# timmeinhardt/trackformer

Measured on AMD Instinct MI355X. Metric: frames/sec, TrackFormer-Deformable inference (ResNet-50, 1333x800, 300 object + 100 track queries, bs 1 per GPU); roofline = ms_deform_attn HBM GB/s, higher is better.
Workload: dtype f32 (dense layers as the fp16 split product on MFMA: two fp16 pieces per activation, three per weight scaled per output channel -- 22 + 1 significand bits per operand, the one dropped product < 2^-22 --, three terms, f32 accumulate)

## Files before the change

include/tf_fused.h:

```cpp
#ifndef TF_FUSED_H_
#define TF_FUSED_H_

#include <stdint.h>

#ifdef __cplusplus
extern "C" {
#endif

int tf_bias_act_f32(float *x, const float *bias, const float *residual, int64_t n, int C, int relu,
                    void *stream);

int tf_add_layernorm_f32(const float *x, const float *res, const float *gamma, const float *beta,
                         float *out, int64_t rows, int C, float eps, void *stream);

int tf_box_refine_f32(const float *delta, const float *ref, float *out, int64_t rows, int ref_dim, float eps, void *stream);

int tf_postprocess_pack_f32(const float *logits, const float *boxes, float *out, int64_t Q, int C, float img_h, float img_w,
                            int clip, void *stream);

int tf_groupnorm_nhwc_f32(const float *x, const float *gamma, const float *beta, float *out, double *workspace, int N,
                          int HW, int C, int G, float eps, int64_t x_image_stride, int64_t out_image_stride, void *stream);
int tf_groupnorm_stats_nhwc_f32(const float *x, double *workspace, int N, int HW, int C, int G, int64_t x_image_stride, void *stream);
int tf_groupnorm_relu_nhwc_f32(const float *x, const float *gamma, const float *beta, float *out, double *workspace, int N,
                               int HW, int C, int G, float eps, int64_t x_image_stride, int64_t out_image_stride, void *stream);
// ... 108 lines not shown
int tf_conv_packed_f32(const float *x, const void *w_packed, const float *bias, const float *residual, float *y, float *workspace,
                       int ksplit, int nimg, int hin, int win, int cin, int cout, int ks, int stride, int relu, int terms,
                       void *stream);
int tf_conv_packed_partials_f32(const float *x, const void *w_packed, const float *bias, float *workspace, int ksplit, int nimg, int hin,
                                int win, int cin, int cout, int ks, int stride, int terms, int *pieces, void *stream);

int tf_linear_res_ln_f32(const float *x, const void *w_packed, const float *bias, const float *residual, const float *ln_weight,
                         const float *ln_bias, float ln_eps, float *y, int64_t M, int K, int N, int terms, void *stream);

int tf_ffn_fused_f32(const float *x, const void *w1_packed, const float *b1, const void *w2_packed, const float *b2,
                     const float *residual, const float *ln_weight, const float *ln_bias, float ln_eps, float *y, int64_t M,
                     int d_model, int d_ffn, int terms, void *stream);

typedef struct tf_proj_group {
    const void *w_packed;
    const float *bias;
    float *y;
    int N;
    int add_x2;
} tf_proj_group;
int tf_linear_groups_f32(const float *x, const float *x2, const tf_proj_group *groups, int ngroups, int64_t M, int K, int terms,
                         void *stream);

int tf_mha_core_f32(const float *q, const float *k, const float *v, float *out, const unsigned char *key_mask,
                    int N, int Lq, int Lk, int H, int D, int ldq, int ldk, int ldv, int ldo, float scale,
                    void *stream);

int tf_mha_core_train_f32(const float *q, const float *k, const float *v, float *out, const unsigned char *key_mask, float *stats,
                          const int64_t *rng, float p, int N, int Lq, int Lk, int H, int D, int ldq, int ldk, int ldv, int ldo,
                          float scale, void *stream);
int tf_mha_core_bwd_f32(const float *dout, const float *q, const float *k, const float *v, const float *out, const float *stats,
                        const unsigned char *key_mask, const int64_t *rng, float p, float *dq, float *dk, float *dv, int N, int Lq,
                        int Lk, int H, int D, int lddo, int ldq, int ldk, int ldv, int ldo, int lddq, int lddk, int lddv, float scale,
                        void *stream);

int tf_nms_host_f32(const float *boxes, const float *scores, int n, float iou_threshold, int64_t *keep, int *n_keep);

#ifdef __cplusplus
}
#endif
#endif
```

include/tf_msda.h:

```cpp
#ifndef TF_MSDA_H_
#define TF_MSDA_H_

#include <stdint.h>

#ifdef __cplusplus
extern "C" {
#endif

#define TF_MSDA_ABI_VERSION 12
#define TF_MSDA_MAX_LEVELS 16

typedef enum tf_msda_status {
    TF_MSDA_OK = 0,
    TF_MSDA_ERR_NULL_POINTER = -1,
    TF_MSDA_ERR_BAD_DIMS = -2,
    TF_MSDA_ERR_SHAPE_SUM = -3,
    TF_MSDA_ERR_LAUNCH = -4,
    TF_MSDA_ERR_NO_DEVICE = -5,
    TF_MSDA_ERR_WORKSPACE = -6
} tf_msda_status;

int tf_msda_abi_version(void);

const char *tf_msda_strerror(int status);

int tf_msda_last_hip_error(void);

const char *tf_msda_last_kernel(void);

int tf_msda_set_tiled(int mode);

int tf_msda_set_option(const char *name, int value);
// ... 79 lines not shown
```

trackformer_amd/build.py:

```python
import hashlib
import os
import shutil
import subprocess
import sys
from concurrent.futures import ThreadPoolExecutor

PKG_DIR = os.path.dirname(os.path.abspath(__file__))
REPO_DIR = os.path.dirname(PKG_DIR)
CSRC = os.path.join(PKG_DIR, "csrc")
LIB_DIR = os.path.join(PKG_DIR, "lib")
INCLUDE = os.path.join(REPO_DIR, "include")
GFX_ARCH = "gfx950"

_TARGETS = [
    ("libtf_msda.so", ["msda_hip.hip", "msda_pquad.hip", "fused_ops.hip", "linear_split.hip", "linear_stream.hip", "mha_core.hip", "ffn_fused.hip", "stem_conv.hip", "msda_host.cpp"], []),
]


def _hipcc():
    exe = shutil.which("hipcc") or "/opt/rocm/bin/hipcc"
    if not os.path.exists(exe):
        raise RuntimeError("hipcc not found (expected on PATH or at /opt/rocm/bin/hipcc)")
    return exe

# ... 37 lines not shown
        src_paths = [os.path.join(CSRC, s) for s in srcs]
        flags = ["--offload-arch=" + GFX_ARCH, "-O3", "-std=c++17", "-fPIC", "-I" + INCLUDE,
                 "-Wno-pass-failed"] + extra
        key = _key(src_paths + headers, flags)
        if not force and not _stale(out, key):
            continue
        obj_dir = os.path.join(LIB_DIR, "obj")
        os.makedirs(obj_dir, exist_ok=True)
        objs = [os.path.join(obj_dir, os.path.splitext(s)[0] + ".o") for s in srcs]
        with ThreadPoolExecutor(max_workers=len(srcs)) as pool:
            list(pool.map(lambda so: _run([_hipcc()] + flags + ["-c", so[0], "-o", so[1]], verbose),
                          zip(src_paths, objs)))
        _run([_hipcc(), "--offload-arch=" + GFX_ARCH, "-shared", "-fPIC", "-pthread"] + objs + ["-o", out], verbose)
        _stamp(out, key)
        built.append(out)
    built += _build_tools(force, verbose)
    return built


def _build_tools(force, verbose):
    out_dir = os.path.join(REPO_DIR, "tools", "bin")
    lib = os.path.join(LIB_DIR, "libtf_msda.so")
    built = []
    for name in ("msda_bench", "linear_bench", "ffn_bench", "proj_groups_bench", "gn_levels_bench"):
        src = os.path.join(REPO_DIR, "tools", name + ".cpp")
        if not os.path.exists(src):
            continue
        os.makedirs(out_dir, exist_ok=True)
        out = os.path.join(out_dir, name)
        flags = ["--offload-arch=" + GFX_ARCH, "-O2", "-std=c++17", "-I" + INCLUDE]
        headers = [os.path.join(INCLUDE, f) for f in os.listdir(INCLUDE) if f.endswith(".h")]
        key = _key([src] + headers, flags)
        if not force and not _stale(out, key) and os.path.getmtime(out) >= os.path.getmtime(lib):
            continue
        _run([_hipcc()] + flags + [src, "-L" + LIB_DIR, "-ltf_msda",
                                   "-Wl,-rpath,$ORIGIN/../../trackformer_amd/lib", "-o", out], verbose)
        _stamp(out, key)
        built.append(out)
    return built


if __name__ == "__main__":
    res = build_all(force="--force" in sys.argv, verbose=True)
    print("built:" if res else "up to date", *res)
```

trackformer_amd/csrc/ffn_fused.hip:

```cpp
#include <hip/hip_runtime.h>

#include <stdint.h>
#include <stdlib.h>

#include <type_traits>

#include "host_dispatch.h"
#include "launch_status.h"
#include "msda_common.h"
#include "split_product.h"
#include "tf_fused.h"
#include "tf_msda.h"

namespace {

template <int D>
struct Geo {
    static_assert(D == 256 || D == 288, "hidden sizes of the reference's configurations");
    static constexpr int NW = D == 256 ? 4 : 3;
    static constexpr int NT = NW * 64;
    static constexpr int TJ = D / 32 / NW;
    static constexpr int XS = D + 8;
    static constexpr int CH = NW * 32;
    static constexpr int HS = CH + 8;
// ... 654 lines not shown
        }
#pragma unroll 1
        for (int k = 0; k < pg.nchunk[ph][1]; ++k, ++ci) {
            const ChunkW nxt = chunk_of(pg.chunk[min(ci + 1, total - 1)]);
            run_chunk(std::true_type{}, cur, nxt, pg.chunk[ci]);
            cur = nxt;
        }
    }
}

template <int SP, int TI>
int launch_groups(const float *x, const float *x2, int M, const ProjGroups &pg, hipStream_t s)
{
    constexpr size_t tile = linln_lds_bytes<256>(TI, Split<SP>::NA), lds_max = tile + 2 * 4 * kMaxProjCols;
    static_assert(lds_max <= 160 * 1024, "the activation tile and the tables do not fit the LDS of a CU");
    const size_t lds = tile + 2 * 4 * (size_t)pg.ncols;
    const void *fn = (const void *)&linear_groups_kernel<SP, TI>;
    if (lds_max > 64 * 1024 && !tfm::raise_dynamic_lds_limit(fn)) return tfm::record_hip(hipErrorInvalidValue);
    const int blocks = (M + 32 * TI - 1) / (32 * TI);
    void *argv[] = {(void *)&x, (void *)&x2, (void *)&M, (void *)&pg};
    return tfm::record_hip(hipLaunchKernel(fn, dim3((unsigned)blocks), dim3(256), argv, lds, s));
}

}

extern "C" int tf_linear_groups_f32(const float *x, const float *x2, const tf_proj_group *groups, int ngroups, int64_t M, int K, int terms,
                                    void *stream)
{
    if (!x || !groups) return TF_MSDA_ERR_NULL_POINTER;
    if (ngroups < 1 || ngroups > kMaxProjGroups) return TF_MSDA_ERR_BAD_DIMS;
    for (int i = 0; i < ngroups; ++i)
        if (!groups[i].w_packed || !groups[i].y || (groups[i].add_x2 && !x2)) return TF_MSDA_ERR_NULL_POINTER;
    const int sp = split_scheme(terms);
    if (M <= 0 || K != 256 || sp == 0 || (M + 128) * (int64_t)K * 4 > 0xFFFFFFFFLL) return TF_MSDA_ERR_BAD_DIMS;
    uintptr_t al = reinterpret_cast<uintptr_t>(x) | reinterpret_cast<uintptr_t>(x2);
    ProjGroups pg{};
    for (int pass = 0; pass < 2; ++pass)
        for (int i = 0; i < ngroups; ++i) {
            const tf_proj_group &g = groups[i];
            if ((g.add_x2 != 0) != (pass == 1)) continue;
            if (g.N <= 0 || (g.N % 32) != 0 || (M + 128) * (int64_t)g.N * 4 > 0xFFFFFFFFLL) return TF_MSDA_ERR_BAD_DIMS;
            al |= reinterpret_cast<uintptr_t>(g.w_packed) | reinterpret_cast<uintptr_t>(g.bias) | reinterpret_cast<uintptr_t>(g.y);
            pg.g[pg.ng++] = ProjGroup{static_cast<const u32x4 *>(g.w_packed), g.bias, g.y, g.N, pg.ncols};
            pg.ncols += (g.N + 255) / 256 * 256;
            if (pass == 0) pg.nplain = pg.ng;
        }
    if ((al & 15) || pg.ncols > kMaxProjCols) return TF_MSDA_ERR_BAD_DIMS;
    int nc = 0;
    for (int ph = 0; ph < 2; ++ph)
        for (int half = 0; half < 2; ++half)
            for (int gi = ph ? pg.nplain : 0; gi < (ph ? pg.ng : pg.nplain); ++gi) {
                const int N = pg.g[gi].N, full_end = N / 256 * 256;
                for (int col0 = half ? full_end : 0; col0 < (half ? N : full_end); col0 += half ? 128 : 256) {
                    pg.chunk[nc++] = gi << 16 | half << 15 | col0 / 128;
                    ++pg.nchunk[ph][half];
                }
            }
    hipStream_t s = static_cast<hipStream_t>(stream);
    if (sp == 3) return launch_groups<3, 1>(x, x2, (int)M, pg, s);
    const int forced = tfm::dense_knob(tfm::kKnobGroupsTi);
    switch (forced ? forced : (M < 4096 ? 1 : 3)) {
    case 1: return launch_groups<16, 1>(x, x2, (int)M, pg, s);
    case 2: return launch_groups<16, 2>(x, x2, (int)M, pg, s);
    default: return launch_groups<16, 3>(x, x2, (int)M, pg, s);
    }
}

extern "C" int tf_linear_res_ln_f32(const float *x, const void *w_packed, const float *bias, const float *residual,
                                    const float *ln_weight, const float *ln_bias, float ln_eps, float *y, int64_t M, int K, int N,
                                    int terms, void *stream)
{
    if (!x || !w_packed || !y) return TF_MSDA_ERR_NULL_POINTER;
    if ((ln_weight == nullptr) != (ln_bias == nullptr)) return TF_MSDA_ERR_NULL_POINTER;
    const int sp = split_scheme(terms);
    if (M <= 0 || K != N || (K != 256 && K != 288) || (M + 128) * (int64_t)K * 4 > 0xFFFFFFFFLL || sp == 0) return TF_MSDA_ERR_BAD_DIMS;
    uintptr_t al = reinterpret_cast<uintptr_t>(x) | reinterpret_cast<uintptr_t>(w_packed) | reinterpret_cast<uintptr_t>(y) |
                   reinterpret_cast<uintptr_t>(bias) | reinterpret_cast<uintptr_t>(residual) | reinterpret_cast<uintptr_t>(ln_weight) |
                   reinterpret_cast<uintptr_t>(ln_bias);
    if (al & 15) return TF_MSDA_ERR_BAD_DIMS;
    const u32x4 *w = static_cast<const u32x4 *>(w_packed);
// ... 1 lines not shown
    return K == 256 ? dispatch_linln_scheme<256>(sp, x, w, bias, residual, ln_weight, ln_bias, ln_eps, y, (int)M, s)
                    : dispatch_linln_scheme<288>(sp, x, w, bias, residual, ln_weight, ln_bias, ln_eps, y, (int)M, s);
}

extern "C" int tf_ffn_fused_f32(const float *x, const void *w1_packed, const float *b1, const void *w2_packed, const float *b2,
                                const float *residual, const float *ln_weight, const float *ln_bias, float ln_eps, float *y,
                                int64_t M, int d_model, int d_ffn, int terms, void *stream)
{
    if (!x || !w1_packed || !w2_packed || !y) return TF_MSDA_ERR_NULL_POINTER;
    if ((ln_weight == nullptr) != (ln_bias == nullptr)) return TF_MSDA_ERR_NULL_POINTER;
    const int sp = split_scheme(terms);
    if (M <= 0 || (d_model != 256 && d_model != 288) || d_ffn <= 0 || sp == 0 ||
        (M + 128) * (int64_t)d_model * 4 > 0xFFFFFFFFLL)
        return TF_MSDA_ERR_BAD_DIMS;
    uintptr_t al = reinterpret_cast<uintptr_t>(x) | reinterpret_cast<uintptr_t>(w1_packed) | reinterpret_cast<uintptr_t>(w2_packed) |
                   reinterpret_cast<uintptr_t>(y) | reinterpret_cast<uintptr_t>(b1) | reinterpret_cast<uintptr_t>(b2) |
                   reinterpret_cast<uintptr_t>(residual) | reinterpret_cast<uintptr_t>(ln_weight) | reinterpret_cast<uintptr_t>(ln_bias);
    if (al & 15) return TF_MSDA_ERR_BAD_DIMS;
    const u32x4 *w1 = static_cast<const u32x4 *>(w1_packed), *w2 = static_cast<const u32x4 *>(w2_packed);
    hipStream_t s = static_cast<hipStream_t>(stream);
    return d_model == 256 ? dispatch_ffn_scheme<256>(sp, x, w1, b1, w2, b2, residual, ln_weight, ln_bias, ln_eps, y, (int)M, d_ffn, s)
                          : dispatch_ffn_scheme<288>(sp, x, w1, b1, w2, b2, residual, ln_weight, ln_bias, ln_eps, y, (int)M, d_ffn, s);
}
```

trackformer_amd/deformable_transformer.py:

```python
import copy
import math

import torch
import torch.nn.functional as F
from torch import nn
from torch.nn.init import constant_, normal_, xavier_uniform_

from . import fused
from .msda import MSDeformAttn, attach_host_shapes
from .nested import inverse_sigmoid, is_all_valid


def _inference(module) -> bool:
    return (not module.training) and (not torch.is_grad_enabled())


def _ffn_hidden(linear, activation, x, inference):
    if inference and activation is F.relu and x.is_cuda and x.dtype == torch.float32:
        if fused.split_linear_enabled():
            y = fused.linear(x, linear.weight, linear.bias, relu=True)
            if y is not None:
                return y
        x2 = x.reshape(-1, x.shape[-1])
        y = torch._addmm_activation(linear.bias, x2, linear.weight.t(), use_gelu=False)
# ... 308 lines not shown
            return (hs, memory, init_reference_out, inter_references, enc_outputs_class,
                    enc_outputs_coord_unact)
        return hs, memory, init_reference_out, inter_references, None, None


class DeformableTransformerEncoderLayer(nn.Module):
    def __init__(self, d_model=256, d_ffn=1024, dropout=0.1, activation="relu", n_levels=4,
                 n_heads=8, n_points=4):
        super().__init__()
        self.self_attn = MSDeformAttn(d_model, n_levels, n_heads, n_points)
        self.dropout1 = nn.Dropout(dropout)
        self.norm1 = nn.LayerNorm(d_model)
        self.linear1 = nn.Linear(d_model, d_ffn)
        self.activation = _get_activation_fn(activation)
        self.dropout2 = nn.Dropout(dropout)
        self.linear2 = nn.Linear(d_ffn, d_model)
        self.dropout3 = nn.Dropout(dropout)
        self.norm2 = nn.LayerNorm(d_model)

    @staticmethod
    def with_pos_embed(tensor, pos):
        return tensor if pos is None else tensor + pos

    def forward_ffn(self, src):
        inf = _inference(self)
        if inf and fused.ffn_fused_enabled() and self.activation is F.relu:
            out = fused.ffn(src, self.linear1, self.linear2, self.norm2, residual=src)
            if out is not None:
                return out
        src2 = fused.module_linear(self.linear2, _ffn_hidden_dropped(self.linear1, self.activation, src, inf, self.dropout2), inf)
        return fused.residual_norm(src, src2, self.norm2, inf, dropout=self.dropout3)

    def forward(self, src, pos, reference_points, spatial_shapes, padding_mask=None):
        inf = _inference(self)
        q, q_pos = (src, pos) if (inf and pos is not None and fused.pos_add_fused_enabled()) else (self.with_pos_embed(src, pos), None)
        if inf and fused.linear_ln_fused_enabled():
            src = self.self_attn(q, reference_points, src, spatial_shapes, padding_mask,
                                 residual_norm=(src, self.norm1), query_pos=q_pos)
            return self.forward_ffn(src)
        src2 = self.self_attn(q, reference_points, src, spatial_shapes, padding_mask, query_pos=q_pos)
        src = fused.residual_norm(src, src2, self.norm1, _inference(self), dropout=self.dropout1)
        return self.forward_ffn(src)


class DeformableTransformerEncoder(nn.Module):
    def __init__(self, encoder_layer, num_layers):
        super().__init__()
        self.layers = _get_clones(encoder_layer, num_layers)
        self.num_layers = num_layers

    @staticmethod
    def get_reference_points(spatial_shapes, valid_ratios, device):
        if torch.is_tensor(spatial_shapes):
            spatial_shapes = _host_shapes(spatial_shapes)
        per_level = []
        for lvl, (h, w) in enumerate(spatial_shapes):
            ys = torch.linspace(0.5, h - 0.5, h, dtype=torch.float32, device=device)
            xs = torch.linspace(0.5, w - 0.5, w, dtype=torch.float32, device=device)
            ref_y, ref_x = torch.meshgrid(ys, xs, indexing="ij")
            ref_y = ref_y.reshape(-1)[None] / (valid_ratios[:, None, lvl, 1] * h)
            ref_x = ref_x.reshape(-1)[None] / (valid_ratios[:, None, lvl, 0] * w)
            per_level.append(torch.stack((ref_x, ref_y), -1))
        reference_points = torch.cat(per_level, 1)
        return reference_points[:, :, None] * valid_ratios[:, None]

    def forward(self, src, spatial_shapes, valid_ratios, pos=None, padding_mask=None,
                unit_ratios=False):
        reference_points = _GEOMETRY.encoder_reference_points(
            _host_shapes(spatial_shapes), valid_ratios, unit_ratios)
        output = src
        for layer in self.layers:
            output = layer(output, pos, reference_points, spatial_shapes, padding_mask)
        return output


class DeformableTransformerDecoderLayer(nn.Module):
    def __init__(self, d_model=256, d_ffn=1024, dropout=0.1, activation="relu", n_levels=4,
                 n_heads=8, n_points=4):
        super().__init__()
        self.cross_attn = MSDeformAttn(d_model, n_levels, n_heads, n_points)
        self.dropout1 = nn.Dropout(dropout)
        self.norm1 = nn.LayerNorm(d_model)
        self.self_attn = nn.MultiheadAttention(d_model, n_heads, dropout=dropout)
        self.dropout2 = nn.Dropout(dropout)
        self.norm2 = nn.LayerNorm(d_model)
        self.linear1 = nn.Linear(d_model, d_ffn)
        self.activation = _get_activation_fn(activation)
        self.dropout3 = nn.Dropout(dropout)
        self.linear2 = nn.Linear(d_ffn, d_model)
        self.dropout4 = nn.Dropout(dropout)
        self.norm3 = nn.LayerNorm(d_model)

    @staticmethod
    def with_pos_embed(tensor, pos):
        return tensor if pos is None else tensor + pos
# ... 173 lines not shown
```

trackformer_amd/fused.py:

```python
import ctypes
import os
import threading

import torch
import torch.nn.functional as F

from . import _cabi


def _stream(device):
    return torch.cuda.current_stream(device).cuda_stream


def _param_ok(t, x):
    return (t.device == x.device and t.dtype == torch.float32 and t.is_contiguous()
            and t.data_ptr() % 16 == 0)


_weight_epoch = 0
_route_epoch = 0


def weight_epoch():
    return _weight_epoch
# ... 610 lines not shown
    if (a.data_ptr() | _ptr(b)) & 15:
        return None
    cols = 0
    for w, bias, _add in groups:
        if not (w.dtype == torch.float32 and w.dim() == 2 and w.is_contiguous() and w.device == x.device and w.shape[1] == K
                and w.shape[0] % 32 == 0 and (M + 128) * w.shape[0] * 4 <= 0xFFFFFFFF):
            return None
        if bias is not None and not (_param_ok(bias, x) and bias.numel() == w.shape[0]):
            return None
        cols += (w.shape[0] + 255) // 256 * 256
    if cols > 4096:
        return None
    packed = [_packed_weight(w, None) for w, _b, _add in groups]
    if any(p is None for p in packed):
        return None
    descs = (_cabi.ProjGroup * len(groups))()
    with torch.cuda.device(x.device):
        ys = [torch.empty((M, w.shape[0]), dtype=torch.float32, device=x.device) for w, _b, _add in groups]
        for d, (w, bias, add), p, y in zip(descs, groups, packed, ys):
            d.w_packed, d.bias, d.y, d.N, d.add_x2 = p.data_ptr(), (bias.data_ptr() if bias is not None else None), y.data_ptr(), w.shape[0], int(bool(add))
        rc = _cabi.lib().tf_linear_groups_f32(a.data_ptr(), _ptr(b) or None, descs, len(groups), M, K, _terms(), _stream(x.device))
    _cabi.check(rc, "tf_linear_groups_f32")
    return [y.view(*x.shape[:-1], y.shape[1]) for y in ys]


def conv3x3(x, w_taps, bias, relu, stride):
    if not (_split_linear and x.is_cuda and x.dtype == torch.float32 and x.dim() == 4
            and x.is_contiguous(memory_format=torch.channels_last) and w_taps.dtype == torch.float32
            and w_taps.dim() == 2 and w_taps.is_contiguous() and w_taps.device == x.device):
        return None
    n, cin, h, w = x.shape
    cout = w_taps.shape[0]
    ks = 3 if w_taps.shape[1] == 9 * cin else 1
    if w_taps.shape[1] != ks * ks * cin or cin % 32 or stride not in (1, 2) or x.numel() == 0:
        return None
    if bias is not None and not (bias.dtype == torch.float32 and bias.is_contiguous() and bias.numel() == cout
                                 and bias.device == x.device):
        return None
    pad = 1 if ks == 3 else 0
    ho, wo = (h + 2 * pad - ks) // stride + 1, (w + 2 * pad - ks) // stride + 1
    cin_ok = cin % 64 == 0 or (ks == 3 and stride == 1 and _conv_halo and cin % 32 == 0)
    stream_route = (_conv_stream and _conv_stream_wins(n * ho * wo, cout) and cin_ok and not (x.data_ptr() & 15)
                    and n * h * w * cin * 4 < 0xC0000000 and (n * ho * wo + 256) * cout * 4 < 0xC0000000)
    halo = ks == 3 and stride == 1 and _conv_halo and stream_route
    ksplit = _conv_ksplit(n * ho * wo, ks * ks * cin, cout, _HALO_KSPLIT_POLICY if halo else None)
    if ks == 1 and (ksplit < _CONV1X1_MIN_PIECES or not _conv1x1_splitk):
# ... 1317 lines not shown
```

trackformer_amd/msda.py:

```python
import ctypes
import math

import torch
import torch.nn.functional as F
from torch import nn
from torch.autograd import Function
from torch.autograd.function import once_differentiable
from torch.nn.init import constant_, xavier_uniform_

from . import _cabi, fused

import os as _os

FUSED_INFERENCE = _os.environ.get("TF_MSDA_FUSED", "1") != "0"

_HOST_SHAPE_ATTR = "_tf_msda_host_shapes"
_shape_array_cache = {}


def attach_host_shapes(spatial_shapes, host_shapes):
    setattr(spatial_shapes, _HOST_SHAPE_ATTR, tuple((int(h), int(w)) for h, w in host_shapes))
    return spatial_shapes


# ... 356 lines not shown
        self.output_proj = nn.Linear(d_model, d_model)
        self._cat_proj = _CatProjection()
        self._reset_parameters()

    def _reset_parameters(self):
        with torch.no_grad():
            constant_(self.sampling_offsets.weight, 0.)
        dirs = [(a, b) for a in (-1, 0, 1) for b in (-1, 0, 1) if (a, b) != (0, 0)]
        if self.n_heads != len(dirs):
            raise ValueError("MSDeformAttn bias initialisation requires n_heads == 8")
        grid = torch.tensor(dirs, dtype=torch.float32).view(self.n_heads, 1, 1, 2)
        grid = grid.repeat(1, self.n_levels, self.n_points, 1)
        scale = torch.arange(1, self.n_points + 1, dtype=torch.float32).view(1, 1, -1, 1)
        with torch.no_grad():
            self.sampling_offsets.bias = nn.Parameter((grid * scale).reshape(-1))
            constant_(self.attention_weights.weight, 0.)
            constant_(self.attention_weights.bias, 0.)
            xavier_uniform_(self.value_proj.weight)
            constant_(self.value_proj.bias, 0.)
            xavier_uniform_(self.output_proj.weight)
            constant_(self.output_proj.bias, 0.)

    def forward(self, query, reference_points, input_flatten, input_spatial_shapes,
                input_padding_mask=None, query_attn_mask=None, residual_norm=None, query_pos=None, value=None):
        if residual_norm is not None:
            out = self._forward(query, reference_points, input_flatten, input_spatial_shapes, input_padding_mask,
                                query_attn_mask, residual_norm, query_pos, value)
            if isinstance(out, _Normed):
                return out.value
            return fused.residual_norm(residual_norm[0], out, residual_norm[1], True)
        return self._forward(query, reference_points, input_flatten, input_spatial_shapes, input_padding_mask, query_attn_mask,
                             None, query_pos, value)

    def _forward(self, query, reference_points, input_flatten, input_spatial_shapes, input_padding_mask, query_attn_mask,
                 residual_norm, query_pos=None, value=None):
        N, Len_q, _ = query.shape
        N, Len_in, _ = input_flatten.shape
        hs = _host_shapes_of(input_spatial_shapes)
        if hs is not None:
            if sum(h * w for h, w in hs) != Len_in:
                raise AssertionError("sum of H_l*W_l does not match the flattened input length")
        else:
            assert (input_spatial_shapes[:, 0] * input_spatial_shapes[:, 1]).sum() == Len_in

        M, L, P = self.n_heads, self.n_levels, self.n_points
        inference = not self.training and not torch.is_grad_enabled()
        fused_inference = (FUSED_INFERENCE and hs is not None and query_attn_mask is None and inference
                           and reference_points.shape[-1] in (2, 4) and (self.d_model // M) % 4 == 0 and P in (1, 2, 4, 8))
        qproj = None
        if value is not None and not inference:
            raise ValueError("MSDeformAttn: a precomputed `value` is an inference-path extension")
        if (value is None and fused_inference and query_pos is not None and input_flatten is query and fused.proj_groups_enabled("enc")
                and fused.pos_add_fused_enabled()):
            w, b = self._cat_proj.get(self)
            ys = fused.linear_groups(query, query_pos, [(self.value_proj.weight, self.value_proj.bias, False), (w, b, True)])
            if ys is not None:
                value, qproj = ys
        if value is None:
            value = fused.module_linear(self.value_proj, input_flatten, inference)
        if input_padding_mask is not None:
            value = value.masked_fill(input_padding_mask[..., None], float(0))
        value = value.view(N, Len_in, M, self.d_model // M)

        if fused_inference and value.is_cuda and value.dtype == torch.float32:
            w, b = self._cat_proj.get(self)
            if qproj is None and query_pos is not None:
                qproj = fused.linear_add(query, query_pos, w, b)
                if qproj is None:
                    query = query + query_pos
            if qproj is None:
                qproj = fused.linear(query, w, b) if fused.split_linear_enabled() else None
            if qproj is None:
                qproj = F.linear(query, w, b)
            output = ms_deform_attn_forward_fused(value, input_spatial_shapes, reference_points,
# ... 43 lines not shown
```

Baseline: 390.9.

## Fuse encoder FFN with next layer's value and query projections

Adds a kernel that runs the encoder layer's FFN plus residual LayerNorm and then, from the still-resident output tile, computes the next layer's value projection and the pos-added offset/attention projections. The encoder loop hands these outputs to the next layer, so each layer no longer launches a separate projection kernel or re-reads its input from HBM. In exchange the kernel is more complex, holds more live state and reuses the hidden-tile LDS for its tables, and it only applies to the 256-wide, 16-term geometry in inference.

```diff
diff --git a/include/tf_fused.h b/include/tf_fused.h
--- a/include/tf_fused.h
+++ b/include/tf_fused.h
@@ -154,6 +154,10 @@
 int tf_linear_groups_f32(const float *x, const float *x2, const tf_proj_group *groups, int ngroups, int64_t M, int K, int terms,
                          void *stream);
 
+int tf_ffn_groups_f32(const float *x, const void *w1_packed, const float *b1, const void *w2_packed, const float *b2,
+                      const float *residual, const float *ln_weight, const float *ln_bias, float ln_eps, float *y, int64_t M,
+                      int d_model, int d_ffn, const float *x2, const tf_proj_group *groups, int ngroups, int terms, void *stream);
+
 int tf_mha_core_f32(const float *q, const float *k, const float *v, float *out, const unsigned char *key_mask,
                     int N, int Lq, int Lk, int H, int D, int ldq, int ldk, int ldv, int ldo, float scale,
                     void *stream);
diff --git a/include/tf_msda.h b/include/tf_msda.h
--- a/include/tf_msda.h
+++ b/include/tf_msda.h
@@ -7,7 +7,7 @@
 extern "C" {
 #endif
 
-#define TF_MSDA_ABI_VERSION 12
+#define TF_MSDA_ABI_VERSION 13
 #define TF_MSDA_MAX_LEVELS 16
 
 typedef enum tf_msda_status {
diff --git a/trackformer_amd/build.py b/trackformer_amd/build.py
--- a/trackformer_amd/build.py
+++ b/trackformer_amd/build.py
@@ -83,7 +83,7 @@
     out_dir = os.path.join(REPO_DIR, "tools", "bin")
     lib = os.path.join(LIB_DIR, "libtf_msda.so")
     built = []
-    for name in ("msda_bench", "linear_bench", "ffn_bench", "proj_groups_bench", "gn_levels_bench"):
+    for name in ("msda_bench", "linear_bench", "ffn_bench", "proj_groups_bench", "ffn_groups_bench", "gn_levels_bench"):
         src = os.path.join(REPO_DIR, "tools", name + ".cpp")
         if not os.path.exists(src):
             continue
diff --git a/trackformer_amd/csrc/ffn_fused.hip b/trackformer_amd/csrc/ffn_fused.hip
--- a/trackformer_amd/csrc/ffn_fused.hip
+++ b/trackformer_amd/csrc/ffn_fused.hip
@@ -700,19 +700,364 @@
     return tfm::record_hip(hipLaunchKernel(fn, dim3((unsigned)blocks), dim3(256), argv, lds, s));
 }
 
-}
-
-extern "C" int tf_linear_groups_f32(const float *x, const float *x2, const tf_proj_group *groups, int ngroups, int64_t M, int K, int terms,
-                                    void *stream)
-{
-    if (!x || !groups) return TF_MSDA_ERR_NULL_POINTER;
-    if (ngroups < 1 || ngroups > kMaxProjGroups) return TF_MSDA_ERR_BAD_DIMS;
-    for (int i = 0; i < ngroups; ++i)
-        if (!groups[i].w_packed || !groups[i].y || (groups[i].add_x2 && !x2)) return TF_MSDA_ERR_NULL_POINTER;
-    const int sp = split_scheme(terms);
-    if (M <= 0 || K != 256 || sp == 0 || (M + 128) * (int64_t)K * 4 > 0xFFFFFFFFLL) return TF_MSDA_ERR_BAD_DIMS;
-    uintptr_t al = reinterpret_cast<uintptr_t>(x) | reinterpret_cast<uintptr_t>(x2);
-    ProjGroups pg{};
+template <int SP, int D, int TI>
+__global__ void __launch_bounds__(Geo<D>::NT, 1)
+ffn_groups_kernel(const float *__restrict__ X, const u32x4 *__restrict__ W1p, const float *__restrict__ b1,
+                  const u32x4 *__restrict__ W2p, const float *__restrict__ b2, const float *R,
+                  const float *__restrict__ gamma, const float *__restrict__ beta, float eps, float *Y, int M, int F,
+                  const float *__restrict__ X2, const ProjGroups pg)
+{
+    using G = Geo<D>;
+    static_assert(SP == 16 && D == 256 && TI == 3, "the flagship geometry only");
+    constexpr int BM = TI * 32, TJ = G::TJ, NW = G::NW, XS = G::XS, HS = G::HS, RING = G::RING, UPC = G::UPC, U1 = G::U1, U2 = G::U2;
+    constexpr int NA = Split<SP>::NA, NB = Split<SP>::NB, US = G::us(NB);
+    constexpr bool F16 = Split<SP>::F16;
+    extern __shared__ __attribute__((aligned(16))) unsigned short s_f[];
+    unsigned short *const sX = s_f;
+    unsigned short *const sH = s_f + NA * BM * XS;
+    const int tid = threadIdx.x, lane = tid & 63;
+    const int wave = __builtin_amdgcn_readfirstlane(tid >> 6);
+    const int m0 = blockIdx.x * BM;
+    const int nchunks = (F + G::CH - 1) / G::CH, KQ2 = F >> 4;
+    const int ntiles1 = (F + 255) / 256 * 8;
+
+    u32x4 ring[RING][US];
+    auto load_unit = [&](int c, auto uc, u32x4 (&dst)[US]) {
+        constexpr int u = decltype(uc)::value;
+        if constexpr (u < U1) {
+            const u32x4 *base = W1p + ((size_t)min(c * NW + wave, ntiles1 - 1) * G::KQ1 * NB + u * 2 * NB) * 64 + lane;
+#pragma unroll
+            for (int i = 0; i < 2 * NB; ++i) dst[i] = base[i * 64];
+        } else {
+            const int q = min(c * U2 + (u - U1), KQ2 - 1);
+#pragma unroll
+            for (int j = 0; j < TJ; ++j)
+#pragma unroll
+                for (int p = 0; p < NB; ++p) dst[j * NB + p] = W2p[(((size_t)(TJ * wave + j) * KQ2 + q) * NB + p) * 64 + lane];
+        }
+    };
+    static_for<G::AHEAD>([&](auto uc) { load_unit(0, uc, ring[decltype(uc)::value]); });
+    __builtin_amdgcn_sched_barrier(0);
+    stage_rows<SP, D, TI>(X, M, m0, sX, tid);
+    __syncthreads();
+
+    f32x16 accy[TI][TJ];
+#pragma unroll
+    for (int i = 0; i < TI; ++i)
+#pragma unroll
+        for (int j = 0; j < TJ; ++j)
+#pragma unroll
+            for (int e = 0; e < 16; ++e) accy[i][j][e] = 0.f;
+
+    const float *const r1 = reinterpret_cast<const float *>(W1p + (size_t)ntiles1 * G::KQ1 * NB * 64);
+    const float *const r2 = reinterpret_cast<const float *>(W2p + (size_t)((D + 255) / 256 * 8) * KQ2 * NB * 64);
+    const int frow = (lane & 31), fk = (lane >> 5) * 8;
+    const int xoff = frow * XS + fk, hoff = frow * HS + fk;
+
+    const __amdgpu_buffer_rsrc_t b1rs = __builtin_amdgcn_make_buffer_rsrc(const_cast<float *>(b1 ? b1 : X), 0, b1 ? (unsigned)F * 4u : 0u, 0x00020000);
+    const __amdgpu_buffer_rsrc_t b2rs = __builtin_amdgcn_make_buffer_rsrc(const_cast<float *>(b2 ? b2 : X), 0, b2 ? (unsigned)D * 4u : 0u, 0x00020000);
+    const unsigned bytes = (unsigned)((size_t)M * D * 4);
+    const __amdgpu_buffer_rsrc_t yrs = __builtin_amdgcn_make_buffer_rsrc(Y, 0, bytes, 0x00020000);
+    const __amdgpu_buffer_rsrc_t rrs = __builtin_amdgcn_make_buffer_rsrc(const_cast<float *>(R ? R : X), 0, R ? bytes : 0u, 0x00020000);
+    const int cbase = wave * (32 * TJ) + 4 * (lane >> 5);
+    f32x4 v[TI][TJ][4];
+
+    for (int c = 0; c < nchunks; ++c) {
+        const int cn = min(c + 1, nchunks - 1);
+        f32x4 b1v[4], r1v[4];
+#pragma unroll
+        for (int g = 0; g < 4; ++g) {
+            r1v[g] = f32x4{1.f, 1.f, 1.f, 1.f};
+            b1v[g] = __builtin_bit_cast(f32x4, __builtin_amdgcn_raw_buffer_load_b128(
+                                                   b1rs, (unsigned)(c * G::CH + wave * 32 + 8 * g + 4 * (lane >> 5)) * 4u, 0, 0));
+            if constexpr (F16)
+                r1v[g] = *reinterpret_cast<const f32x4 *>(r1 + min(c * G::CH + wave * 32 + 8 * g + 4 * (lane >> 5), ntiles1 * 32 - 4));
+        }
+        if (c == nchunks - 1) {
+#pragma unroll
+            for (int i = 0; i < TI; ++i)
+#pragma unroll
+                for (int j = 0; j < TJ; ++j)
+#pragma unroll
+                    for (int g = 0; g < 4; ++g)
+                        v[i][j][g] = __builtin_bit_cast(f32x4, __builtin_amdgcn_raw_buffer_load_b128(
+                                                                   rrs, (unsigned)((m0 + i * 32 + frow) * D + cbase + 32 * j + 8 * g) * 4u, 0, 0));
+        }
+        f32x16 acch[TI][1];
+#pragma unroll
+        for (int i = 0; i < TI; ++i)
+#pragma unroll
+            for (int e = 0; e < 16; ++e) acch[i][0][e] = 0.f;
+
+        auto prefetch = [&](auto uc) {
+            constexpr int ahead = decltype(uc)::value + G::AHEAD;
+            if constexpr (ahead < UPC) load_unit(c, std::integral_constant<int, ahead>{}, ring[ahead % RING]);
+            else load_unit(cn, std::integral_constant<int, ahead - UPC>{}, ring[ahead % RING]);
+        };
+        u32x4 xf[2][TI][NA];
+        auto read_x = [&](auto stc) {
+            constexpr int st = decltype(stc)::value;
+#pragma unroll
+            for (int i = 0; i < TI; ++i)
+#pragma unroll
+                for (int p = 0; p < NA; ++p)
+                    xf[st & 1][i][p] = *reinterpret_cast<const u32x4 *>(&sX[(p * BM + i * 32) * XS + xoff + st * 16]);
+        };
+        read_x(std::integral_constant<int, 0>{});
+        static_for<G::KQ1>([&](auto stc) {
+            constexpr int st = decltype(stc)::value;
+            if constexpr ((st & 1) == 0) prefetch(std::integral_constant<int, st / 2>{});
+            if constexpr (st + 1 < G::KQ1) read_x(std::integral_constant<int, st + 1>{});
+            __builtin_amdgcn_sched_barrier(0);
+            const u32x4 (&cur)[US] = ring[(st / 2) % RING];
+            u32x4 wf[1][NB];
+#pragma unroll
+            for (int p = 0; p < NB; ++p) wf[0][p] = cur[(st & 1) * NB + p];
+            mfma_tiles<SP, TI, 1, false>(acch, xf[st & 1], wf);
+        });
+
+        __syncthreads();
+        const int hcol = c * G::CH + wave * 32 + 4 * (lane >> 5);
+#pragma unroll
+        for (int i = 0; i < TI; ++i)
+#pragma unroll
+            for (int g = 0; g < 4; ++g) {
+                f32x4 hv;
+#pragma unroll
+                for (int e = 0; e < 4; ++e) {
+                    const float t = F16 ? __builtin_fmaf(acch[i][0][4 * g + e], r1v[g][e], b1v[g][e]) : acch[i][0][4 * g + e] + b1v[g][e];
+                    hv[e] = (t < 0.f || hcol + 8 * g >= F) ? 0.f : t;
+                }
+                u32x2 pc[NA];
+                split4<SP>(hv, pc);
+                const int o = (i * 32 + frow) * HS + wave * 32 + 8 * g + 4 * (lane >> 5);
+#pragma unroll
+                for (int p = 0; p < NA; ++p) *reinterpret_cast<u32x2 *>(&sH[p * BM * HS + o]) = pc[p];
+            }
+        __syncthreads();
+
+        u32x4 hf[2][TI][NA];
+        auto read_h = [&](auto vc) {
+            constexpr int kv = decltype(vc)::value;
+#pragma unroll
+            for (int i = 0; i < TI; ++i)
+#pragma unroll
+                for (int p = 0; p < NA; ++p)
+                    hf[kv & 1][i][p] = *reinterpret_cast<const u32x4 *>(&sH[(p * BM + i * 32) * HS + hoff + kv * 16]);
+        };
+        read_h(std::integral_constant<int, 0>{});
+        static_for<U2>([&](auto vc) {
+            constexpr int kv = decltype(vc)::value;
+            prefetch(std::integral_constant<int, U1 + kv>{});
+            if constexpr (kv + 1 < U2) read_h(std::integral_constant<int, kv + 1>{});
+            __builtin_amdgcn_sched_barrier(0);
+            const u32x4 (&cur)[US] = ring[(U1 + kv) % RING];
+            u32x4 wf[TJ][NB];
+#pragma unroll
+            for (int j = 0; j < TJ; ++j)
+#pragma unroll
+                for (int p = 0; p < NB; ++p) wf[j][p] = cur[j * NB + p];
+            mfma_tiles<SP, TI, TJ, false>(accy, hf[kv & 1], wf);
+        });
+    }
+    rows_epilogue<D, TI, true, F16>(accy, v, b2rs, r2, gamma, beta, eps, yrs, reinterpret_cast<float *>(sH), m0, wave, lane);
+
+    constexpr int KQ = G::KQ1, GAHEAD = RING - 2;
+    static_assert(RING == linln_ring(TI) && US == 2 * NB && KQ % RING == 0 && (KQ / 2) % RING == 0 && GAHEAD <= KQ / 2,
+                  "the projection chunks run on the feed-forward block's ring; a chunk starts at ring slot 0");
+    constexpr int kRedFloats = 2 * NW * BM;
+    static_assert((kRedFloats + 2 * kMaxProjCols + NW * 1024) * 4 <= BM * HS * 2 * NA, "the tables and the waves' store tiles do not fit the hidden tile");
+    float *const sBias = reinterpret_cast<float *>(sH) + kRedFloats;
+    float *const sScale = sBias + pg.ncols;
+    float *const sT = reinterpret_cast<float *>(sH) + BM * HS * NA / 2 - (NW - wave) * 1024;
+
+    auto chunk_of = [&](int code) {
+        const ProjGroup &g = pg.g[code >> 16];
+        const int col0 = (code & 0x7fff) * 128;
+        ChunkW c;
+        c.half = (code >> 15) & 1;
+        const int tile = (col0 >> 5) + (c.half ? wave : 2 * wave);
+        c.base = g.w + (size_t)tile * (KQ * NB * 64) + lane;
+        c.us = c.half ? 2 * NB : NB;
+        c.as = c.half ? NB : KQ * NB;
+        return c;
+    };
+    auto load_gunit = [&](const ChunkW &c, auto uc, u32x4 (&dst)[US]) {
+        constexpr int u = decltype(uc)::value;
+        const u32x4 *p0 = c.base + (size_t)(u * c.us) * 64;
+#pragma unroll
+        for (int a = 0; a < 2; ++a)
+#pragma unroll
+            for (int p = 0; p < NB; ++p) dst[a * NB + p] = p0[(size_t)(a * c.as + p) * 64];
+    };
+    u32x4 yf[2][TI][NA];
+    auto read_y = [&](auto stc) {
+        constexpr int st = decltype(stc)::value;
+#pragma unroll
+        for (int i = 0; i < TI; ++i)
+#pragma unroll
+            for (int p = 0; p < NA; ++p)
+                yf[st & 1][i][p] = *reinterpret_cast<const u32x4 *>(&sX[(p * BM + i * 32) * XS + xoff + st * 16]);
+    };
+    auto run_chunk = [&](auto halfc, const ChunkW &cur, const ChunkW &nxt, int code) {
+        constexpr bool HALF = decltype(halfc)::value;
+        constexpr int CJ = HALF ? 1 : 2, UNITS = HALF ? KQ / 2 : KQ;
+        const ProjGroup &g = pg.g[code >> 16];
+        const int col0 = (code & 0x7fff) * 128;
+        const int N = g.N;
+        const int wcol = col0 + wave * (32 * CJ);
+        f32x16 acc[TI][CJ];
+#pragma unroll
+        for (int i = 0; i < TI; ++i)
+#pragma unroll
+            for (int j = 0; j < CJ; ++j)
+#pragma unroll
+                for (int e = 0; e < 16; ++e) acc[i][j][e] = 0.f;
+        read_y(std::integral_constant<int, 0>{});
+        static_for<KQ>([&](auto stc) {
+            constexpr int st = decltype(stc)::value;
+            constexpr int u = HALF ? st / 2 : st;
+            if constexpr (!HALF || (st & 1) == 0) {
+                constexpr int ahead = u + GAHEAD;
+                if constexpr (ahead < UNITS) load_gunit(cur, std::integral_constant<int, ahead>{}, ring[ahead % RING]);
+                else load_gunit(nxt, std::integral_constant<int, ahead - UNITS>{}, ring[ahead % RING]);
+            }
+            if constexpr (st + 1 < KQ) read_y(std::integral_constant<int, st + 1>{});
+            __builtin_amdgcn_sched_barrier(0);
+            const u32x4 (&cu)[US] = ring[u % RING];
+            u32x4 wf[CJ][NB];
+#pragma unroll
+            for (int j = 0; j < CJ; ++j)
+#pragma unroll
+                for (int p = 0; p < NB; ++p) wf[j][p] = cu[(HALF ? (st & 1) : j) * NB + p];
+            mfma_tiles<SP, TI, CJ, false>(acc, yf[st & 1], wf);
+        });
+        const unsigned ybytes = (unsigned)((size_t)M * N * 4);
+        const int trow = lane >> 3, tg = lane & 7;
+#pragma unroll
+        for (int j = 0; j < CJ; ++j) {
+            const __amdgpu_buffer_rsrc_t grs = __builtin_amdgcn_make_buffer_rsrc(g.y, 0, wcol + 32 * j < N ? ybytes : 0u, 0x00020000);
+            f32x4 bv[4], rv[4];
+#pragma unroll
+            for (int q = 0; q < 4; ++q) {
+                const int col = wcol + 32 * j + 8 * q + 4 * (lane >> 5);
+                bv[q] = *reinterpret_cast<const f32x4 *>(sBias + g.cbase + col);
+                rv[q] = f32x4{1.f, 1.f, 1.f, 1.f};
+                if constexpr (F16) rv[q] = *reinterpret_cast<const f32x4 *>(sScale + g.cbase + col);
+            }
+#pragma unroll
+            for (int i = 0; i < TI; ++i) {
+                __builtin_amdgcn_fence(__ATOMIC_RELEASE, "wavefront");
+#pragma unroll
+                for (int q = 0; q < 4; ++q) {
+                    f32x4 o;
+#pragma unroll
+                    for (int e = 0; e < 4; ++e) o[e] = F16 ? __builtin_fmaf(acc[i][j][4 * q + e], rv[q][e], bv[q][e]) : acc[i][j][4 * q + e] + bv[q][e];
+                    *reinterpret_cast<f32x4 *>(sT + frow * 32 + ((2 * q + (lane >> 5)) ^ (frow & 7)) * 4) = o;
+                }
+                __builtin_amdgcn_fence(__ATOMIC_ACQ_REL, "wavefront");
+                __builtin_amdgcn_wave_barrier();
+#pragma unroll
+                for (int t = 0; t < 4; ++t) {
+                    const f32x4 o = *reinterpret_cast<const f32x4 *>(sT + (8 * t + trow) * 32 + (tg ^ trow) * 4);
+                    __builtin_amdgcn_raw_buffer_store_b128(__builtin_bit_cast(u32x4, o), grs,
+                                                           (unsigned)((m0 + i * 32 + 8 * t + trow) * N + wcol + 32 * j + 4 * tg) * 4u, 0, tfm::kStoreAux);
+                }
+            }
+        }
+    };
+    auto stage_y = [&](auto addc) {
+        constexpr bool ADD = decltype(addc)::value;
+        f32x4 p2[ADD ? TI : 1][TJ][4];
+        if constexpr (ADD) {
+            const __amdgpu_buffer_rsrc_t x2rs = __builtin_amdgcn_make_buffer_rsrc(const_cast<float *>(X2 ? X2 : X), 0, X2 ? bytes : 0u, 0x00020000);
+            __builtin_amdgcn_s_waitcnt(0x0F70);
+            __builtin_amdgcn_sched_barrier(0);
+#pragma unroll
+            for (int i = 0; i < TI; ++i)
+#pragma unroll
+                for (int j = 0; j < TJ; ++j)
+#pragma unroll
+                    for (int g = 0; g < 4; ++g) {
+                        const unsigned off = (unsigned)((m0 + i * 32 + frow) * D + cbase + 32 * j + 8 * g) * 4u;
+                        v[i][j][g] = __builtin_bit_cast(f32x4, __builtin_amdgcn_raw_buffer_load_b128(yrs, off, 0, 0));
+                        p2[i][j][g] = __builtin_bit_cast(f32x4, __builtin_amdgcn_raw_buffer_load_b128(x2rs, off, 0, 0));
+                    }
+            __builtin_amdgcn_sched_barrier(0);
+        }
+#pragma unroll
+        for (int i = 0; i < TI; ++i)
+#pragma unroll
+            for (int j = 0; j < TJ; ++j)
+#pragma unroll
+                for (int g = 0; g < 4; ++g) {
+                    f32x4 yv = v[i][j][g];
+                    if constexpr (ADD) yv += p2[i][j][g];
+                    u32x2 pc[NA];
+                    split4<SP>(yv, pc);
+#pragma unroll
+                    for (int p = 0; p < NA; ++p)
+                        *reinterpret_cast<u32x2 *>(&sX[(p * BM + i * 32 + frow) * XS + cbase + 32 * j + 8 * g]) = pc[p];
+                }
+    };
+
+    const int total = pg.nchunk[0][0] + pg.nchunk[0][1] + pg.nchunk[1][0] + pg.nchunk[1][1];
+    int ci = 0;
+    ChunkW cur = chunk_of(pg.chunk[0]);
+    static_for<GAHEAD>([&](auto uc) { load_gunit(cur, uc, ring[decltype(uc)::value]); });
+    __builtin_amdgcn_sched_barrier(0);
+    for (int gq = 0; gq < pg.ng; ++gq) {
+        const ProjGroup &g = pg.g[gq];
+        const int npad = (g.N + 255) / 256 * 256;
+        const float *const r = reinterpret_cast<const float *>(g.w + (size_t)(npad / 32) * KQ * NB * 64);
+        const __amdgpu_buffer_rsrc_t brs =
+            __builtin_amdgcn_make_buffer_rsrc(const_cast<float *>(g.bias ? g.bias : X), 0, g.bias ? (unsigned)g.N * 4u : 0u, 0x00020000);
+        for (int c = tid * 4; c < npad; c += 4 * G::NT) {
+            *reinterpret_cast<f32x4 *>(sBias + g.cbase + c) = __builtin_bit_cast(f32x4, __builtin_amdgcn_raw_buffer_load_b128(brs, (unsigned)c * 4u, 0, 0));
+            if constexpr (F16) *reinterpret_cast<f32x4 *>(sScale + g.cbase + c) = *reinterpret_cast<const f32x4 *>(r + c);
+        }
+    }
+#pragma unroll 1
+    for (int ph = 0; ph < 2; ++ph) {
+        if ((ph ? pg.ng - pg.nplain : pg.nplain) == 0) continue;
+        if (ph == 1) {
+            if (pg.nplain > 0) __syncthreads();
+            stage_y(std::true_type{});
+        } else {
+            stage_y(std::false_type{});
+        }
+        __syncthreads();
+#pragma unroll 1
+        for (int k = 0; k < pg.nchunk[ph][0]; ++k, ++ci) {
+            const ChunkW nxt = chunk_of(pg.chunk[min(ci + 1, total - 1)]);
+            run_chunk(std::false_type{}, cur, nxt, pg.chunk[ci]);
+            cur = nxt;
+        }
+#pragma unroll 1
+        for (int k = 0; k < pg.nchunk[ph][1]; ++k, ++ci) {
+            const ChunkW nxt = chunk_of(pg.chunk[min(ci + 1, total - 1)]);
+            run_chunk(std::true_type{}, cur, nxt, pg.chunk[ci]);
+            cur = nxt;
+        }
+    }
+}
+
+int launch_ffn_groups(const float *x, const u32x4 *w1, const float *b1, const u32x4 *w2, const float *b2, const float *res,
+                      const float *gamma, const float *beta, float eps, float *y, int M, int F, const float *x2, const ProjGroups &pg,
+                      hipStream_t s)
+{
+    constexpr size_t lds = ffn_lds_bytes<256>(3, Split<16>::NA);
+    static_assert(lds <= 160 * 1024, "the two tiles do not fit the LDS of a CU");
+    const void *fn = (const void *)&ffn_groups_kernel<16, 256, 3>;
+    if (!tfm::raise_dynamic_lds_limit(fn)) return tfm::record_hip(hipErrorInvalidValue);
+    const int blocks = (M + 95) / 96;
+    void *argv[] = {(void *)&x, (void *)&w1, (void *)&b1, (void *)&w2, (void *)&b2, (void *)&res, (void *)&gamma,
+                    (void *)&beta, (void *)&eps, (void *)&y, (void *)&M, (void *)&F, (void *)&x2, (void *)&pg};
+    return tfm::record_hip(hipLaunchKernel(fn, dim3((unsigned)blocks), dim3(Geo<256>::NT), argv, lds, s));
+}
+
+int make_proj_groups(const tf_proj_group *groups, int ngroups, int64_t M, ProjGroups &pg, uintptr_t &al)
+{
     for (int pass = 0; pass < 2; ++pass)
         for (int i = 0; i < ngroups; ++i) {
             const tf_proj_group &g = groups[i];
@@ -723,7 +1068,7 @@
             pg.ncols += (g.N + 255) / 256 * 256;
             if (pass == 0) pg.nplain = pg.ng;
         }
-    if ((al & 15) || pg.ncols > kMaxProjCols) return TF_MSDA_ERR_BAD_DIMS;
+    if (pg.ncols > kMaxProjCols) return TF_MSDA_ERR_BAD_DIMS;
     int nc = 0;
     for (int ph = 0; ph < 2; ++ph)
         for (int half = 0; half < 2; ++half)
@@ -734,6 +1079,24 @@
                     ++pg.nchunk[ph][half];
                 }
             }
+    return TF_MSDA_OK;
+}
+
+}
+
+extern "C" int tf_linear_groups_f32(const float *x, const float *x2, const tf_proj_group *groups, int ngroups, int64_t M, int K, int terms,
+                                    void *stream)
+{
+    if (!x || !groups) return TF_MSDA_ERR_NULL_POINTER;
+    if (ngroups < 1 || ngroups > kMaxProjGroups) return TF_MSDA_ERR_BAD_DIMS;
+    for (int i = 0; i < ngroups; ++i)
+        if (!groups[i].w_packed || !groups[i].y || (groups[i].add_x2 && !x2)) return TF_MSDA_ERR_NULL_POINTER;
+    const int sp = split_scheme(terms);
+    if (M <= 0 || K != 256 || sp == 0 || (M + 128) * (int64_t)K * 4 > 0xFFFFFFFFLL) return TF_MSDA_ERR_BAD_DIMS;
+    uintptr_t al = reinterpret_cast<uintptr_t>(x) | reinterpret_cast<uintptr_t>(x2);
+    ProjGroups pg{};
+    if (int rc = make_proj_groups(groups, ngroups, M, pg, al)) return rc;
+    if (al & 15) return TF_MSDA_ERR_BAD_DIMS;
     hipStream_t s = static_cast<hipStream_t>(stream);
     if (sp == 3) return launch_groups<3, 1>(x, x2, (int)M, pg, s);
     const int forced = tfm::dense_knob(tfm::kKnobGroupsTi);
@@ -781,3 +1144,26 @@
     return d_model == 256 ? dispatch_ffn_scheme<256>(sp, x, w1, b1, w2, b2, residual, ln_weight, ln_bias, ln_eps, y, (int)M, d_ffn, s)
                           : dispatch_ffn_scheme<288>(sp, x, w1, b1, w2, b2, residual, ln_weight, ln_bias, ln_eps, y, (int)M, d_ffn, s);
 }
+
+extern "C" int tf_ffn_groups_f32(const float *x, const void *w1_packed, const float *b1, const void *w2_packed, const float *b2,
+                                 const float *residual, const float *ln_weight, const float *ln_bias, float ln_eps, float *y, int64_t M,
+                                 int d_model, int d_ffn, const float *x2, const tf_proj_group *groups, int ngroups, int terms, void *stream)
+{
+    if (!x || !w1_packed || !w2_packed || !y || !groups) return TF_MSDA_ERR_NULL_POINTER;
+    if ((ln_weight == nullptr) != (ln_bias == nullptr)) return TF_MSDA_ERR_NULL_POINTER;
+    if (ngroups < 1 || ngroups > kMaxProjGroups) return TF_MSDA_ERR_BAD_DIMS;
+    for (int i = 0; i < ngroups; ++i)
+        if (!groups[i].w_packed || !groups[i].y || (groups[i].add_x2 && !x2)) return TF_MSDA_ERR_NULL_POINTER;
+    if (M <= 0 || d_model != 256 || terms != 16 || !ln_weight || d_ffn < Geo<256>::CH || (d_ffn & 15) ||
+        (M + 128) * (int64_t)d_model * 4 > 0xFFFFFFFFLL)
+        return TF_MSDA_ERR_BAD_DIMS;
+    uintptr_t al = reinterpret_cast<uintptr_t>(x) | reinterpret_cast<uintptr_t>(w1_packed) | reinterpret_cast<uintptr_t>(w2_packed) |
+                   reinterpret_cast<uintptr_t>(y) | reinterpret_cast<uintptr_t>(b1) | reinterpret_cast<uintptr_t>(b2) |
+                   reinterpret_cast<uintptr_t>(residual) | reinterpret_cast<uintptr_t>(ln_weight) | reinterpret_cast<uintptr_t>(ln_bias) |
+                   reinterpret_cast<uintptr_t>(x2);
+    ProjGroups pg{};
+    if (int rc = make_proj_groups(groups, ngroups, M, pg, al)) return rc;
+    if (al & 15) return TF_MSDA_ERR_BAD_DIMS;
+    return launch_ffn_groups(x, static_cast<const u32x4 *>(w1_packed), b1, static_cast<const u32x4 *>(w2_packed), b2, residual, ln_weight,
+                             ln_bias, ln_eps, y, (int)M, d_ffn, x2, pg, static_cast<hipStream_t>(stream));
+}
diff --git a/trackformer_amd/deformable_transformer.py b/trackformer_amd/deformable_transformer.py
--- a/trackformer_amd/deformable_transformer.py
+++ b/trackformer_amd/deformable_transformer.py
@@ -354,25 +354,33 @@
     def with_pos_embed(tensor, pos):
         return tensor if pos is None else tensor + pos
 
-    def forward_ffn(self, src):
+    def forward_ffn(self, src, pos=None, next_attn=None):
         inf = _inference(self)
         if inf and fused.ffn_fused_enabled() and self.activation is F.relu:
+            if (next_attn is not None and pos is not None and fused.ffn_proj_fused_enabled() and fused.pos_add_fused_enabled()
+                    and fused.proj_groups_enabled("enc")):
+                w, b = next_attn._cat_proj.get(next_attn)
+                out = fused.ffn_groups(src, self.linear1, self.linear2, self.norm2, src, pos,
+                                       [(next_attn.value_proj.weight, next_attn.value_proj.bias, False), (w, b, True)])
+                if out is not None:
+                    return out[0], out[1][0], out[1][1]
             out = fused.ffn(src, self.linear1, self.linear2, self.norm2, residual=src)
             if out is not None:
-                return out
+                return out if next_attn is None else (out, None, None)
         src2 = fused.module_linear(self.linear2, _ffn_hidden_dropped(self.linear1, self.activation, src, inf, self.dropout2), inf)
-        return fused.residual_norm(src, src2, self.norm2, inf, dropout=self.dropout3)
-
-    def forward(self, src, pos, reference_points, spatial_shapes, padding_mask=None):
+        out = fused.residual_norm(src, src2, self.norm2, inf, dropout=self.dropout3)
+        return out if next_attn is None else (out, None, None)
+
+    def forward(self, src, pos, reference_points, spatial_shapes, padding_mask=None, next_attn=None, value=None, qproj=None):
         inf = _inference(self)
         q, q_pos = (src, pos) if (inf and pos is not None and fused.pos_add_fused_enabled()) else (self.with_pos_embed(src, pos), None)
         if inf and fused.linear_ln_fused_enabled():
             src = self.self_attn(q, reference_points, src, spatial_shapes, padding_mask,
-                                 residual_norm=(src, self.norm1), query_pos=q_pos)
-            return self.forward_ffn(src)
-        src2 = self.self_attn(q, reference_points, src, spatial_shapes, padding_mask, query_pos=q_pos)
+                                 residual_norm=(src, self.norm1), query_pos=q_pos, value=value, qproj=qproj)
+            return self.forward_ffn(src, pos, next_attn)
+        src2 = self.self_attn(q, reference_points, src, spatial_shapes, padding_mask, query_pos=q_pos, value=value, qproj=qproj)
         src = fused.residual_norm(src, src2, self.norm1, _inference(self), dropout=self.dropout1)
-        return self.forward_ffn(src)
+        return self.forward_ffn(src, pos, next_attn)
 
 
 class DeformableTransformerEncoder(nn.Module):
@@ -401,8 +409,15 @@
         reference_points = _GEOMETRY.encoder_reference_points(
             _host_shapes(spatial_shapes), valid_ratios, unit_ratios)
         output = src
-        for layer in self.layers:
-            output = layer(output, pos, reference_points, spatial_shapes, padding_mask)
+        hand_on = (not self.training and not torch.is_grad_enabled() and pos is not None and fused.ffn_proj_fused_enabled())
+        value = qproj = None
+        for i, layer in enumerate(self.layers):
+            if hand_on:
+                nxt = self.layers[i + 1].self_attn if i + 1 < len(self.layers) else None
+                out = layer(output, pos, reference_points, spatial_shapes, padding_mask, next_attn=nxt, value=value, qproj=qproj)
+                output, value, qproj = out if nxt is not None else (out, None, None)
+            else:
+                output = layer(output, pos, reference_points, spatial_shapes, padding_mask)
         return output
 
 
diff --git a/trackformer_amd/fused.py b/trackformer_amd/fused.py
--- a/trackformer_amd/fused.py
+++ b/trackformer_amd/fused.py
@@ -656,6 +656,81 @@
         rc = _cabi.lib().tf_linear_groups_f32(a.data_ptr(), _ptr(b) or None, descs, len(groups), M, K, _terms(), _stream(x.device))
     _cabi.check(rc, "tf_linear_groups_f32")
     return [y.view(*x.shape[:-1], y.shape[1]) for y in ys]
+
+
+_ffn_proj_fused = os.environ.get("TF_FFN_PROJ_FUSED", "1") != "0"
+
+
+def ffn_proj_fused_enabled():
+    return _ffn_proj_fused
+
+
+def set_ffn_proj_fused(on):
+    global _ffn_proj_fused
+    prev, _ffn_proj_fused = _ffn_proj_fused, bool(on)
+    return _switched(prev, _ffn_proj_fused)
+
+
+def ffn_groups(x, linear1, linear2, norm, residual, x2, groups):
+    if not (_ffn_proj_fused and _ffn_fused and _split_linear and x.is_cuda and x.dtype == torch.float32 and _terms() == 16
+            and norm is not None and 1 <= len(groups) <= 8 and x.numel()):
+        return None
+    if _n_six_term_routes or debug_checks_active():
+        return None
+    w1, w2 = linear1.weight, linear2.weight
+    F_, D = w1.shape
+    if D != 256 or x.shape[-1] != D or tuple(w2.shape) != (D, F_) or F_ % 16 or F_ < 128:
+        return None
+    if not all(w.dtype == torch.float32 and w.is_contiguous() and w.device == x.device for w in (w1, w2)):
+        return None
+    if not (norm.elementwise_affine and tuple(norm.normalized_shape) == (D,)):
+        return None
+    if not all(v is None or _param_ok(v, x) for v in (linear1.bias, linear2.bias, norm.weight, norm.bias)):
+        return None
+    a = x.reshape(-1, D)
+    a = a if a.is_contiguous() else a.contiguous()
+    M = a.shape[0]
+    if M < max(_FFN_FUSED_MIN_ROWS, _PROJ_GROUPS_MIN_ROWS) or (M + 128) * D * 4 > 0xFFFFFFFF:
+        return None
+    res = None
+    if residual is not None:
+        if residual.dtype != torch.float32 or residual.device != x.device or residual.numel() != a.numel():
+            return None
+        res = residual.reshape(-1, D)
+        res = res if res.is_contiguous() else res.contiguous()
+    b = None
+    if any(add for _w, _b, add in groups):
+        if x2 is None or x2.dtype != torch.float32 or x2.shape != x.shape or x2.device != x.device:
+            return None
+        b = x2.reshape(-1, D)
+        b = b if b.is_contiguous() else b.contiguous()
+    if (a.data_ptr() | _ptr(res) | _ptr(b)) & 15:
+        return None
+    cols = 0
+    for w, bias, _add in groups:
+        if not (w.dtype == torch.float32 and w.dim() == 2 and w.is_contiguous() and w.device == x.device and w.shape[1] == D
+                and w.shape[0] % 32 == 0 and (M + 128) * w.shape[0] * 4 <= 0xFFFFFFFF):
+            return None
+        if bias is not None and not (_param_ok(bias, x) and bias.numel() == w.shape[0]):
+            return None
+        cols += (w.shape[0] + 255) // 256 * 256
+    if cols > 4096:
+        return None
+    p1, p2 = _packed_weight(w1, None), _packed_weight(w2, None)
+    packed = [_packed_weight(w, None) for w, _b, _add in groups]
+    if p1 is None or p2 is None or any(p is None for p in packed):
+        return None
+    descs = (_cabi.ProjGroup * len(groups))()
+    with torch.cuda.device(x.device):
+        y = torch.empty((M, D), dtype=torch.float32, device=x.device)
+        ys = [torch.empty((M, w.shape[0]), dtype=torch.float32, device=x.device) for w, _b, _add in groups]
+        for d, (w, bias, add), p, yg in zip(descs, groups, packed, ys):
+            d.w_packed, d.bias, d.y, d.N, d.add_x2 = p.data_ptr(), (bias.data_ptr() if bias is not None else None), yg.data_ptr(), w.shape[0], int(bool(add))
+        rc = _cabi.lib().tf_ffn_groups_f32(a.data_ptr(), p1.data_ptr(), _ptr(linear1.bias) or None, p2.data_ptr(), _ptr(linear2.bias) or None,
+                                           _ptr(res) or None, norm.weight.data_ptr(), norm.bias.data_ptr(), float(norm.eps), y.data_ptr(),
+                                           M, D, F_, _ptr(b) or None, descs, len(groups), 16, _stream(x.device))
+    _cabi.check(rc, "tf_ffn_groups_f32")
+    return y.view(x.shape), [yg.view(*x.shape[:-1], yg.shape[1]) for yg in ys]
 
 
 def conv3x3(x, w_taps, bias, relu, stride):
diff --git a/trackformer_amd/msda.py b/trackformer_amd/msda.py
--- a/trackformer_amd/msda.py
+++ b/trackformer_amd/msda.py
@@ -402,18 +402,18 @@
             constant_(self.output_proj.bias, 0.)
 
     def forward(self, query, reference_points, input_flatten, input_spatial_shapes,
-                input_padding_mask=None, query_attn_mask=None, residual_norm=None, query_pos=None, value=None):
+                input_padding_mask=None, query_attn_mask=None, residual_norm=None, query_pos=None, value=None, qproj=None):
         if residual_norm is not None:
             out = self._forward(query, reference_points, input_flatten, input_spatial_shapes, input_padding_mask,
-                                query_attn_mask, residual_norm, query_pos, value)
+                                query_attn_mask, residual_norm, query_pos, value, qproj)
             if isinstance(out, _Normed):
                 return out.value
             return fused.residual_norm(residual_norm[0], out, residual_norm[1], True)
         return self._forward(query, reference_points, input_flatten, input_spatial_shapes, input_padding_mask, query_attn_mask,
-                             None, query_pos, value)
+                             None, query_pos, value, qproj)
 
     def _forward(self, query, reference_points, input_flatten, input_spatial_shapes, input_padding_mask, query_attn_mask,
-                 residual_norm, query_pos=None, value=None):
+                 residual_norm, query_pos=None, value=None, qproj=None):
         N, Len_q, _ = query.shape
         N, Len_in, _ = input_flatten.shape
         hs = _host_shapes_of(input_spatial_shapes)
@@ -427,9 +427,10 @@
         inference = not self.training and not torch.is_grad_enabled()
         fused_inference = (FUSED_INFERENCE and hs is not None and query_attn_mask is None and inference
                            and reference_points.shape[-1] in (2, 4) and (self.d_model // M) % 4 == 0 and P in (1, 2, 4, 8))
-        qproj = None
-        if value is not None and not inference:
-            raise ValueError("MSDeformAttn: a precomputed `value` is an inference-path extension")
+        if (value is not None or qproj is not None) and not inference:
+            raise ValueError("MSDeformAttn: a precomputed `value` / `qproj` is an inference-path extension")
+        if not fused_inference:
+            qproj = None
         if (value is None and fused_inference and query_pos is not None and input_flatten is query and fused.proj_groups_enabled("enc")
                 and fused.pos_add_fused_enabled()):
             w, b = self._cat_proj.get(self)
```

New measurement: 385.1. -1.5%, worse.
